# vita-epfl/CrowdNav

Measured on NVIDIA H100. Metric: env-steps/sec at 5 humans × batched envs; 500-case success/collision parity, higher is better.
Workload: dtype f64 state + f32 ORCA solver

## Files before the change

crowdnav_b200/csrc/reset_kernel.cu:

```cuda
#include <limits.h>
#include "scene.cuh"

namespace cs {

__device__ __forceinline__ bool next_seed(const crowdsim_reset_args &a, int e, const int *assigned, uint32_t &seed, int &case_id)
{
    if (a.case_counter) {
        const int c = assigned ? assigned[e] : atomicAdd(a.case_counter, 1);
        if (c >= a.case_total) return false;
        seed = queue_seed(a, c); case_id = c;
        return true;
    }
    seed = a.seed[e];
    if (a.seed_stride) a.seed[e] = seed + a.seed_stride;
    case_id = -1;
    return true;
}

struct ResetKArgs {
    crowdsim_reset_args a;
    crowdsim_state st;
    crowdsim_episodes ep;
    crowdsim_autoreset ar;
    int has_ep, B, N;
    int *assigned;
};

__device__ __forceinline__ void reset_env(const ResetKArgs &A, int e, MT &rng)
{
    const crowdsim_reset_args &a = A.a;
    const int N = A.N;
    uint32_t seed; int case_id;
    if (!next_seed(a, e, A.assigned, seed, case_id)) {
        if (A.st.active) A.st.active[e] = 0;
        if (A.has_ep) A.ep.ep_case[e] = -1;
        return;
    }
    rng.seed(seed);
    double *hp = A.st.h_pos + (size_t)e * N * 2, *hv = A.st.h_vel + (size_t)e * N * 2;
    double *hg = A.st.h_goal + (size_t)e * N * 2, *ha = A.st.h_attr + (size_t)e * N * 2;
    st2(A.st.r_pos, e, make_double2(0.0, -a.circle_radius)); st2(A.st.r_goal, e, make_double2(0.0, a.circle_radius));
    st2(A.st.r_vel, e, make_double2(0, 0)); st2(A.st.r_attr, e, make_double2(a.robot_radius, a.robot_v_pref));
    if (A.st.r_theta) A.st.r_theta[e] = CS_PI / 2;
    A.st.g_time[e] = 0.0;
    generate_scene(rng, a, N, hp, hg, ha);
    for (int i = 0; i < N; ++i) { hv[2 * i] = 0.0; hv[2 * i + 1] = 0.0; }
    if (A.st.active) A.st.active[e] = 1;
    if (A.has_ep) {
        A.ep.ep_steps[e] = 0; A.ep.ep_return[e] = 0.0; A.ep.ep_too_close[e] = 0; A.ep.ep_min_dist_sum[e] = 0.0;
        if (a.case_counter) A.ep.ep_case[e] = case_id;
    }
}

__device__ __forceinline__ void prefetch_env(const ResetKArgs &A, int e, MT &rng)
{
    const crowdsim_autoreset &ar = A.ar;
    const int N = A.N;
    uint32_t seed; int case_id;
    if (!next_seed(A.a, e, A.assigned, seed, case_id)) {
        ar.n_case[e] = -1;
        st_release_u8(ar.n_state + e, CROWDSIM_SLOT_EXHAUSTED);
        return;
    }
    rng.seed(seed);
    generate_scene(rng, A.a, N, ar.n_h_pos + (size_t)e * N * 2, ar.n_h_goal + (size_t)e * N * 2, ar.n_h_attr + (size_t)e * N * 2);
    ar.n_case[e] = case_id;
    st_release_u8(ar.n_state + e, CROWDSIM_SLOT_READY);
}

template <bool PREFETCH>
__global__ void __launch_bounds__(32, 32) scene_kernel(const __grid_constant__ ResetKArgs A)
{
    CS_RES_BEGIN
    const int lane = threadIdx.x, base = blockIdx.x * 32, e = base + lane;
    const bool need = e < A.B && (PREFETCH ? ld_acquire_u8(A.ar.n_state + e) == (A.assigned ? CROWDSIM_SLOT_CLAIMED : CROWDSIM_SLOT_EMPTY)
                                           : !(A.a.mask && !A.a.mask[e]));
    const unsigned bal = __ballot_sync(0xffffffffu, need);
    MT rng; rng.mt = A.a.scene_mt + base + lane; rng.stride = A.B;
    for (int k = lane; k < __popc(bal); k += 32) {
        const int slot = base + (int)__fns(bal, 0, k + 1);
        if (PREFETCH) prefetch_env(A, slot, rng); else reset_env(A, slot, rng);
    }
#ifdef CS_RESIDENCY_PROBE
    __syncwarp();
#endif
    CS_RES_END(CS_RES_SCENE);
}

constexpr int kAssignThreads = 64;
constexpr int kAssignRun = 32;
template <bool PREFETCH>
__global__ void __launch_bounds__(kAssignThreads, 16) assign_cases_kernel(const __grid_constant__ ResetKArgs A)
{
    CS_RES_BEGIN
    __shared__ int s_warp[kAssignThreads / 32];
    const int tid = threadIdx.x, lane = tid & 31, w = tid >> 5;
    int base = *A.a.case_counter;
    for (int start = 0; start < A.B; start += kAssignThreads * kAssignRun) {
        const int e0 = start + tid * kAssignRun;
        uint8_t flag[kAssignRun];
        #pragma unroll
        for (int j = 0; j < kAssignRun; ++j) {
            const int e = e0 + j;
            flag[j] = 0;
            if (e < A.B) {
                if (PREFETCH) flag[j] = ld_relaxed_u8(A.ar.n_state + e) == CROWDSIM_SLOT_EMPTY;
                else flag[j] = !(A.a.mask && !A.a.mask[e]);
            }
        }
        if (PREFETCH) fence_acquire_gpu();
        unsigned need = 0;
        #pragma unroll
        for (int j = 0; j < kAssignRun; ++j) need |= (unsigned)flag[j] << j;
        const int cnt = __popc(need);
        int incl = cnt;
        #pragma unroll
        for (int d = 1; d < 32; d <<= 1) { const int t = __shfl_up_sync(0xffffffffu, incl, d); if (lane >= d) incl += t; }
        if (lane == 31) s_warp[w] = incl;
        __syncthreads();
        int next = base + incl - cnt;
        #pragma unroll
        for (int v = 0; v < kAssignThreads / 32; ++v) if (v < w) next += s_warp[v];
        int total = 0;
        #pragma unroll
        for (int v = 0; v < kAssignThreads / 32; ++v) total += s_warp[v];
        while (need) {
            const int j = __ffs(need) - 1;
            need &= need - 1u;
            A.assigned[e0 + j] = next++;
            if (PREFETCH) A.ar.n_state[e0 + j] = CROWDSIM_SLOT_CLAIMED;
        }
        base += total;
        __syncthreads();
    }
    if (tid == 0) *A.a.case_counter = base;
    CS_RES_END(CS_RES_ASSIGN);
}

template <bool PREFETCH>
static int launch_scene_kernel(ResetKArgs A, int B, cudaStream_t stream)
{
    cudaError_t err = set_carveout<scene_kernel<PREFETCH>>();
    if (err == cudaSuccess) err = set_carveout<assign_cases_kernel<PREFETCH>>();
    if (err != cudaSuccess) return (int)err;
    A.assigned = nullptr;
    if (A.a.case_counter && (PREFETCH || A.has_ep)) {
        A.assigned = PREFETCH ? A.ar.n_case : A.ep.ep_case;
        assign_cases_kernel<PREFETCH><<<1, kAssignThreads, 0, stream>>>(A);
        ++g_launches;
    }
    scene_kernel<PREFETCH><<<(B + 31) / 32, 32, 0, stream>>>(A);
    ++g_launches;
    return (int)cudaGetLastError();
}

}

#ifdef CS_RESIDENCY_PROBE
extern "C" int crowdsim_residency_probe_refill(cs::ResRec *out, unsigned cap, unsigned *n) { return cs::res_read(out, cap, n); }
#endif

static int check_reset_args(const crowdsim_reset_args *args, int B, int N)
{
    if (!args || B < 0 || N < 0) return CROWDSIM_EINVAL;
    if (!args->case_counter && !args->seed) return CROWDSIM_EINVAL;
    if (N > CROWDSIM_MAX_HUMANS) return CROWDSIM_EUNSUPPORTED;
    if (args->rule != CROWDSIM_RULE_CIRCLE && args->rule != CROWDSIM_RULE_SQUARE && args->rule != CROWDSIM_RULE_MIXED) return CROWDSIM_EUNSUPPORTED;
    if (args->rule == CROWDSIM_RULE_MIXED && N < 5) return CROWDSIM_EUNSUPPORTED;
    if (!args->scene_mt) return CROWDSIM_EINVAL;
    if (B > INT_MAX / 624) return CROWDSIM_EUNSUPPORTED;
    return CROWDSIM_OK;
}

extern "C" int crowdsim_reset(const crowdsim_reset_args *args, int B, int N, crowdsim_state *st, crowdsim_episodes *ep,
                              void *stream)
{
    if (!st) return CROWDSIM_EINVAL;
    if (int rc = check_reset_args(args, B, N)) return rc;
    if (N > 0 && (!st->h_pos || !st->h_vel || !st->h_goal || !st->h_attr)) return CROWDSIM_EINVAL;
    if (!st->r_pos || !st->r_vel || !st->r_goal || !st->r_attr || !st->g_time) return CROWDSIM_EINVAL;
    if (ep && (!ep->ep_steps || !ep->ep_return || !ep->ep_too_close || !ep->ep_min_dist_sum || !ep->ep_case)) return CROWDSIM_EINVAL;
    if (B == 0) return CROWDSIM_OK;
    cs::ResetKArgs A; A.a = *args; A.st = *st; A.has_ep = ep != nullptr; A.B = B; A.N = N;
    if (ep) A.ep = *ep; else memset(&A.ep, 0, sizeof(A.ep));
    memset(&A.ar, 0, sizeof(A.ar));
    return cs::launch_scene_kernel<false>(A, B, (cudaStream_t)stream);
}

extern "C" int crowdsim_prefetch_scenes(const crowdsim_reset_args *args, int B, int N, const crowdsim_autoreset *ar, void *stream)
{
    if (!ar) return CROWDSIM_EINVAL;
    if (int rc = check_reset_args(args, B, N)) return rc;
    if (!ar->n_state || !ar->n_case || !ar->want || (N > 0 && (!ar->n_h_pos || !ar->n_h_goal || !ar->n_h_attr))) return CROWDSIM_EINVAL;
    if (B == 0) return CROWDSIM_OK;
    cs::ResetKArgs A; A.a = *args; A.ar = *ar; A.has_ep = 0; A.B = B; A.N = N;
    memset(&A.st, 0, sizeof(A.st)); memset(&A.ep, 0, sizeof(A.ep));
    return cs::launch_scene_kernel<true>(A, B, (cudaStream_t)stream);
}
```

crowdnav_b200/csrc/scene.cuh:

```cuda
#pragma once
#include "crowdsim_common.cuh"

namespace cs {

struct MT {
    uint32_t *mt;
    int stride;
    int pos;
    bool first;
    uint32_t a, a1, m;
    __host__ __device__ __forceinline__ uint32_t &w(int i) { return mt[i * stride]; }
    static __host__ __device__ __forceinline__ uint32_t init_step(uint32_t s, int k) { return 1812433253u * (s ^ (s >> 30)) + (uint32_t)k; }
    __host__ __device__ void seed(uint32_t s) {
        a = s; a1 = init_step(s, 1);
        m = a1;
        for (int k = 2; k <= 397; ++k) m = init_step(m, k);
        pos = 0; first = true;
    }
    __host__ __device__ __forceinline__ void resume(int p) { pos = p; first = false; }
    __host__ __device__ void store_seeded() {
        if (!first) return;
        for (int i = pos; i < 624; ++i) { w(i) = a; a = init_step(a, i + 1); }
        first = false;
    }
    __host__ __device__ __forceinline__ uint32_t next() {
        const int i = pos;
        const int i1 = (i == 623) ? 0 : i + 1;
        const int im = (i < 227) ? i + 397 : i - 227;
        uint32_t wi, wi1, wm;
        if (first) { wi = a; wi1 = (i == 623) ? w(0) : a1; wm = (i < 227) ? m : w(im); }
        else { wi = w(i); wi1 = w(i1); wm = w(im); }
        const uint32_t y0 = (wi & 0x80000000u) | (wi1 & 0x7fffffffu);
        uint32_t y = wm ^ (y0 >> 1) ^ ((y0 & 1u) ? 0x9908b0dfu : 0u);
        w(i) = y;
        if (first) {
            a = a1; a1 = init_step(a1, i + 2); m = init_step(m, i + 398);
            first = i != 623;
        }
        pos = i1;
        y ^= (y >> 11); y ^= (y << 7) & 0x9d2c5680u; y ^= (y << 15) & 0xefc60000u; y ^= (y >> 18);
        return y;
    }
    __host__ __device__ __forceinline__ double next_double() {
        const uint32_t a_ = next() >> 5, b_ = next() >> 6;
        return (a_ * 67108864.0 + b_) / 9007199254740992.0;
    }
    __host__ __device__ __forceinline__ int next_index(uint32_t A) {
        const uint32_t rng = A - 1u;
        if (rng == 0u) return 0;
        uint32_t mask = rng;
        mask |= mask >> 1; mask |= mask >> 2; mask |= mask >> 4; mask |= mask >> 8; mask |= mask >> 16;
        uint32_t v;
        do { v = next() & mask; } while (v > rng);
        return (int)v;
    }
};

template <class RNG>
__host__ __device__ __forceinline__ void generate_scene(RNG &rng, const crowdsim_reset_args &a, int N, double *hp, double *hg, double *ha)
{
    const double rpx = 0.0, rpy = -a.circle_radius, rgx = 0.0, rgy = a.circle_radius;
    auto put = [&](int i, double px, double py, double gx, double gy, double radius, double v_pref) {
        hp[2 * i] = px; hp[2 * i + 1] = py; hg[2 * i] = gx; hg[2 * i + 1] = gy; ha[2 * i] = radius; ha[2 * i + 1] = v_pref;
    };
    auto attributes = [&](double &radius, double &v_pref) {
        radius = a.human_radius; v_pref = a.human_v_pref;
        if (a.randomize_attributes) {
            v_pref = 0.5 + (1.5 - 0.5) * rng.next_double();
            radius = 0.3 + (0.5 - 0.3) * rng.next_double();
        }
    };
    auto circle_human = [&](int i) {
        double radius, v_pref, px, py; attributes(radius, v_pref);
        for (;;) {
            const double angle = rng.next_double() * CS_PI * 2;
            const double px_noise = (rng.next_double() - 0.5) * v_pref;
            const double py_noise = (rng.next_double() - 0.5) * v_pref;
            px = a.circle_radius * cos(angle) + px_noise;
            py = a.circle_radius * sin(angle) + py_noise;
            bool collide = false;
            for (int k = -1; k < i && !collide; ++k) {
                const double ar = (k < 0) ? a.robot_radius : ha[2 * k];
                const double apx = (k < 0) ? rpx : hp[2 * k], apy = (k < 0) ? rpy : hp[2 * k + 1];
                const double agx = (k < 0) ? rgx : hg[2 * k], agy = (k < 0) ? rgy : hg[2 * k + 1];
                const double min_dist = radius + ar + a.discomfort_dist;
                if (norm2(px - apx, py - apy) < min_dist || norm2(px - agx, py - agy) < min_dist) collide = true;
            }
            if (!collide) break;
        }
        put(i, px, py, -px, -py, radius, v_pref);
    };
    auto square_human = [&](int i) {
        double radius, v_pref, px, py, gx, gy; attributes(radius, v_pref);
        const double sign = (rng.next_double() > 0.5) ? -1.0 : 1.0;
        for (;;) {
            px = rng.next_double() * a.square_width * 0.5 * sign;
            py = (rng.next_double() - 0.5) * a.square_width;
            bool collide = false;
            for (int k = -1; k < i && !collide; ++k) {
                const double ar = (k < 0) ? a.robot_radius : ha[2 * k];
                const double apx = (k < 0) ? rpx : hp[2 * k], apy = (k < 0) ? rpy : hp[2 * k + 1];
                if (norm2(px - apx, py - apy) < radius + ar + a.discomfort_dist) collide = true;
            }
            if (!collide) break;
        }
        for (;;) {
            gx = rng.next_double() * a.square_width * 0.5 * -sign;
            gy = (rng.next_double() - 0.5) * a.square_width;
            bool collide = false;
            for (int k = -1; k < i && !collide; ++k) {
                const double ar = (k < 0) ? a.robot_radius : ha[2 * k];
                const double agx = (k < 0) ? rgx : hg[2 * k], agy = (k < 0) ? rgy : hg[2 * k + 1];
                if (norm2(gx - agx, gy - agy) < radius + ar + a.discomfort_dist) collide = true;
            }
            if (!collide) break;
        }
        put(i, px, py, gx, gy, radius, v_pref);
    };
    if (a.rule == CROWDSIM_RULE_CIRCLE) { for (int i = 0; i < N; ++i) circle_human(i); return; }
    if (a.rule == CROWDSIM_RULE_SQUARE) { for (int i = 0; i < N; ++i) square_human(i); return; }
    const bool is_static = rng.next_double() < 0.2;
    double prob = rng.next_double();
    const double p_static[6] = {0.05, 0.2, 0.2, 0.3, 0.1, 0.15}, p_dynamic[6] = {0.0, 0.3, 0.3, 0.2, 0.1, 0.1};
    int count = N;
    for (int key = is_static ? 0 : 1; key <= 5; ++key) {
        const double value = is_static ? p_static[key] : p_dynamic[key];
        if (prob - value <= 0) { count = key; break; }
        prob -= value;
    }
    if (count > N) count = N;
    int placed = 0;
    if (is_static) {
        const double width = 4, height = 8;
        if (count == 0 && N > 0) { put(0, 0.0, -10.0, 0.0, -10.0, a.human_radius, a.human_v_pref); placed = 1; }
        for (int i = 0; i < count; ++i) {
            const double sign = (rng.next_double() > 0.5) ? -1.0 : 1.0;
            double px, py;
            for (;;) {
                px = rng.next_double() * width * 0.5 * sign;
                py = (rng.next_double() - 0.5) * height;
                bool collide = false;
                for (int k = -1; k < i && !collide; ++k) {
                    const double ar = (k < 0) ? a.robot_radius : ha[2 * k];
                    const double apx = (k < 0) ? rpx : hp[2 * k], apy = (k < 0) ? rpy : hp[2 * k + 1];
                    if (norm2(px - apx, py - apy) < a.human_radius + ar + a.discomfort_dist) collide = true;
                }
                if (!collide) break;
            }
            put(i, px, py, px, py, a.human_radius, a.human_v_pref);
        }
        if (count > 0) placed = count;
    } else {
        for (int i = 0; i < count; ++i) { if (i < 2) circle_human(i); else square_human(i); }
        placed = count;
    }
    for (int i = placed; i < N; ++i) {
        const double x = CROWDSIM_PARKED_X + 100.0 * i;
        put(i, x, CROWDSIM_PARKED_X, x, CROWDSIM_PARKED_X, a.human_radius, a.human_v_pref);
    }
}

__device__ __forceinline__ uint32_t queue_seed(const crowdsim_reset_args &a, int c)
{
    return a.seed_base + (a.case_wrap > 0 ? (uint32_t)(((long long)a.case_first + c) % a.case_wrap) : (uint32_t)c);
}

}
```

Baseline: 1.321 billion.

## Generate scenes in shared-memory scratch with a flattened rejection loop and wider blocks

After: 1.367 billion, median of 6. 3.5% higher.

```diff
diff --git a/crowdnav_b200/csrc/reset_kernel.cu b/crowdnav_b200/csrc/reset_kernel.cu
--- a/crowdnav_b200/csrc/reset_kernel.cu
+++ b/crowdnav_b200/csrc/reset_kernel.cu
@@ -26,7 +26,12 @@
     int *assigned;
 };
 
-__device__ __forceinline__ void reset_env(const ResetKArgs &A, int e, MT &rng)
+__device__ __forceinline__ void store_scene(const double *scratch, int N, double *hp, double *hg, double *ha)
+{
+    for (int j = 0; j < 2 * N; ++j) { hp[j] = scratch[j]; hg[j] = scratch[2 * N + j]; ha[j] = scratch[4 * N + j]; }
+}
+
+__device__ __forceinline__ void reset_env(const ResetKArgs &A, int e, MT &rng, double *scratch)
 {
     const crowdsim_reset_args &a = A.a;
     const int N = A.N;
@@ -43,7 +48,8 @@
     st2(A.st.r_vel, e, make_double2(0, 0)); st2(A.st.r_attr, e, make_double2(a.robot_radius, a.robot_v_pref));
     if (A.st.r_theta) A.st.r_theta[e] = CS_PI / 2;
     A.st.g_time[e] = 0.0;
-    generate_scene(rng, a, N, hp, hg, ha);
+    generate_scene(rng, a, N, scratch, scratch + 2 * N, scratch + 4 * N);
+    store_scene(scratch, N, hp, hg, ha);
     for (int i = 0; i < N; ++i) { hv[2 * i] = 0.0; hv[2 * i + 1] = 0.0; }
     if (A.st.active) A.st.active[e] = 1;
     if (A.has_ep) {
@@ -52,7 +58,7 @@
     }
 }
 
-__device__ __forceinline__ void prefetch_env(const ResetKArgs &A, int e, MT &rng)
+__device__ __forceinline__ void prefetch_env(const ResetKArgs &A, int e, MT &rng, double *scratch)
 {
     const crowdsim_autoreset &ar = A.ar;
     const int N = A.N;
@@ -63,23 +69,36 @@
         return;
     }
     rng.seed(seed);
-    generate_scene(rng, A.a, N, ar.n_h_pos + (size_t)e * N * 2, ar.n_h_goal + (size_t)e * N * 2, ar.n_h_attr + (size_t)e * N * 2);
+    generate_scene(rng, A.a, N, scratch, scratch + 2 * N, scratch + 4 * N);
+    store_scene(scratch, N, ar.n_h_pos + (size_t)e * N * 2, ar.n_h_goal + (size_t)e * N * 2, ar.n_h_attr + (size_t)e * N * 2);
     ar.n_case[e] = case_id;
     st_release_u8(ar.n_state + e, CROWDSIM_SLOT_READY);
 }
 
+constexpr int kSceneSlots = 48;
+static_assert(kSceneSlots >= 32 && kSceneSlots <= 64, "a scene block ballots its slots in two words");
+
+__host__ __device__ __forceinline__ int scene_scratch_stride(int N) { return 6 * N + 1; }
+
 template <bool PREFETCH>
 __global__ void __launch_bounds__(32, 32) scene_kernel(const __grid_constant__ ResetKArgs A)
 {
     CS_RES_BEGIN
-    const int lane = threadIdx.x, base = blockIdx.x * 32, e = base + lane;
-    const bool need = e < A.B && (PREFETCH ? ld_acquire_u8(A.ar.n_state + e) == (A.assigned ? CROWDSIM_SLOT_CLAIMED : CROWDSIM_SLOT_EMPTY)
-                                           : !(A.a.mask && !A.a.mask[e]));
-    const unsigned bal = __ballot_sync(0xffffffffu, need);
+    extern __shared__ double s_scene[];
+    const int lane = threadIdx.x, base = blockIdx.x * kSceneSlots;
+    auto need = [&](int j) {
+        const int e = base + j;
+        if (j >= kSceneSlots || e >= A.B) return false;
+        return PREFETCH ? ld_acquire_u8(A.ar.n_state + e) == (A.assigned ? CROWDSIM_SLOT_CLAIMED : CROWDSIM_SLOT_EMPTY)
+                        : !(A.a.mask && !A.a.mask[e]);
+    };
+    const unsigned lo = __ballot_sync(0xffffffffu, need(lane)), hi = __ballot_sync(0xffffffffu, need(32 + lane));
+    const int n_lo = __popc(lo), n = n_lo + __popc(hi);
     MT rng; rng.mt = A.a.scene_mt + base + lane; rng.stride = A.B;
-    for (int k = lane; k < __popc(bal); k += 32) {
-        const int slot = base + (int)__fns(bal, 0, k + 1);
-        if (PREFETCH) prefetch_env(A, slot, rng); else reset_env(A, slot, rng);
+    double *scratch = s_scene + (size_t)lane * scene_scratch_stride(A.N);
+    for (int k = lane; k < n; k += 32) {
+        const int slot = base + (k < n_lo ? (int)__fns(lo, 0, k + 1) : 32 + (int)__fns(hi, 0, k - n_lo + 1));
+        if (PREFETCH) prefetch_env(A, slot, rng, scratch); else reset_env(A, slot, rng, scratch);
     }
 #ifdef CS_RESIDENCY_PROBE
     __syncwarp();
@@ -149,7 +168,12 @@
         assign_cases_kernel<PREFETCH><<<1, kAssignThreads, 0, stream>>>(A);
         ++g_launches;
     }
-    scene_kernel<PREFETCH><<<(B + 31) / 32, 32, 0, stream>>>(A);
+    const size_t smem = (size_t)32 * scene_scratch_stride(A.N) * sizeof(double);
+    if (smem > 48 * 1024) {
+        err = cudaFuncSetAttribute(scene_kernel<PREFETCH>, cudaFuncAttributeMaxDynamicSharedMemorySize, (int)smem);
+        if (err != cudaSuccess) return (int)err;
+    }
+    scene_kernel<PREFETCH><<<(B + kSceneSlots - 1) / kSceneSlots, 32, smem, stream>>>(A);
     ++g_launches;
     return (int)cudaGetLastError();
 }
diff --git a/crowdnav_b200/csrc/scene.cuh b/crowdnav_b200/csrc/scene.cuh
--- a/crowdnav_b200/csrc/scene.cuh
+++ b/crowdnav_b200/csrc/scene.cuh
@@ -63,96 +63,74 @@
     auto put = [&](int i, double px, double py, double gx, double gy, double radius, double v_pref) {
         hp[2 * i] = px; hp[2 * i + 1] = py; hg[2 * i] = gx; hg[2 * i + 1] = gy; ha[2 * i] = radius; ha[2 * i + 1] = v_pref;
     };
-    auto attributes = [&](double &radius, double &v_pref) {
-        radius = a.human_radius; v_pref = a.human_v_pref;
-        if (a.randomize_attributes) {
-            v_pref = 0.5 + (1.5 - 0.5) * rng.next_double();
-            radius = 0.3 + (0.5 - 0.3) * rng.next_double();
+    bool is_static = false;
+    int count = N, placed = N;
+    if (a.rule == CROWDSIM_RULE_MIXED) {
+        is_static = rng.next_double() < 0.2;
+        double prob = rng.next_double();
+        const double p_static[6] = {0.05, 0.2, 0.2, 0.3, 0.1, 0.15}, p_dynamic[6] = {0.0, 0.3, 0.3, 0.2, 0.1, 0.1};
+        for (int key = is_static ? 0 : 1; key <= 5; ++key) {
+            const double value = is_static ? p_static[key] : p_dynamic[key];
+            if (prob - value <= 0) { count = key; break; }
+            prob -= value;
         }
+        if (count > N) count = N;
+        placed = count;
+        if (is_static && count == 0 && N > 0) { put(0, 0.0, -10.0, 0.0, -10.0, a.human_radius, a.human_v_pref); placed = 1; }
+    }
+    enum { kCircle, kSquare, kStatic };
+    auto kind_of = [&](int i) {
+        if (a.rule == CROWDSIM_RULE_CIRCLE) return (int)kCircle;
+        if (a.rule == CROWDSIM_RULE_SQUARE) return (int)kSquare;
+        return is_static ? (int)kStatic : (i < 2 ? (int)kCircle : (int)kSquare);
     };
-    auto circle_human = [&](int i) {
-        double radius, v_pref, px, py; attributes(radius, v_pref);
-        for (;;) {
+    double radius = 0, v_pref = 0, sign = 0, px = 0, py = 0;
+    auto collides = [&](int i, double x, double y, bool pos, bool goal) {
+        for (int k = -1; k < i; ++k) {
+            const double ar = (k < 0) ? a.robot_radius : ha[2 * k];
+            const double min_dist = radius + ar + a.discomfort_dist;
+            if (pos) {
+                const double apx = (k < 0) ? rpx : hp[2 * k], apy = (k < 0) ? rpy : hp[2 * k + 1];
+                if (norm2(x - apx, y - apy) < min_dist) return true;
+            }
+            if (goal) {
+                const double agx = (k < 0) ? rgx : hg[2 * k], agy = (k < 0) ? rgy : hg[2 * k + 1];
+                if (norm2(x - agx, y - agy) < min_dist) return true;
+            }
+        }
+        return false;
+    };
+    int stage = 0;
+    for (int i = 0; i < count;) {
+        const int kind = kind_of(i);
+        if (stage == 0) {
+            radius = a.human_radius; v_pref = a.human_v_pref;
+            if (kind != kStatic && a.randomize_attributes) {
+                v_pref = 0.5 + (1.5 - 0.5) * rng.next_double();
+                radius = 0.3 + (0.5 - 0.3) * rng.next_double();
+            }
+            if (kind != kCircle) sign = (rng.next_double() > 0.5) ? -1.0 : 1.0;
+            stage = 1;
+        }
+        if (kind == kCircle) {
             const double angle = rng.next_double() * CS_PI * 2;
             const double px_noise = (rng.next_double() - 0.5) * v_pref;
             const double py_noise = (rng.next_double() - 0.5) * v_pref;
-            px = a.circle_radius * cos(angle) + px_noise;
-            py = a.circle_radius * sin(angle) + py_noise;
-            bool collide = false;
-            for (int k = -1; k < i && !collide; ++k) {
-                const double ar = (k < 0) ? a.robot_radius : ha[2 * k];
-                const double apx = (k < 0) ? rpx : hp[2 * k], apy = (k < 0) ? rpy : hp[2 * k + 1];
-                const double agx = (k < 0) ? rgx : hg[2 * k], agy = (k < 0) ? rgy : hg[2 * k + 1];
-                const double min_dist = radius + ar + a.discomfort_dist;
-                if (norm2(px - apx, py - apy) < min_dist || norm2(px - agx, py - agy) < min_dist) collide = true;
+            double sin_a, cos_a;
+            sincos(angle, &sin_a, &cos_a);
+            px = a.circle_radius * cos_a + px_noise;
+            py = a.circle_radius * sin_a + py_noise;
+            if (!collides(i, px, py, true, true)) { put(i, px, py, -px, -py, radius, v_pref); ++i; stage = 0; }
+        } else {
+            const bool goal = stage == 2;
+            const double width = kind == kStatic ? 4.0 : a.square_width, height = kind == kStatic ? 8.0 : a.square_width;
+            const double x = rng.next_double() * width * 0.5 * (goal ? -sign : sign);
+            const double y = (rng.next_double() - 0.5) * height;
+            if (!collides(i, x, y, !goal, goal)) {
+                if (kind == kSquare && !goal) { px = x; py = y; stage = 2; }
+                else { put(i, goal ? px : x, goal ? py : y, x, y, radius, v_pref); ++i; stage = 0; }
             }
-            if (!collide) break;
         }
-        put(i, px, py, -px, -py, radius, v_pref);
-    };
-    auto square_human = [&](int i) {
-        double radius, v_pref, px, py, gx, gy; attributes(radius, v_pref);
-        const double sign = (rng.next_double() > 0.5) ? -1.0 : 1.0;
-        for (;;) {
-            px = rng.next_double() * a.square_width * 0.5 * sign;
-            py = (rng.next_double() - 0.5) * a.square_width;
-            bool collide = false;
-            for (int k = -1; k < i && !collide; ++k) {
-                const double ar = (k < 0) ? a.robot_radius : ha[2 * k];
-                const double apx = (k < 0) ? rpx : hp[2 * k], apy = (k < 0) ? rpy : hp[2 * k + 1];
-                if (norm2(px - apx, py - apy) < radius + ar + a.discomfort_dist) collide = true;
-            }
-            if (!collide) break;
-        }
-        for (;;) {
-            gx = rng.next_double() * a.square_width * 0.5 * -sign;
-            gy = (rng.next_double() - 0.5) * a.square_width;
-            bool collide = false;
-            for (int k = -1; k < i && !collide; ++k) {
-                const double ar = (k < 0) ? a.robot_radius : ha[2 * k];
-                const double agx = (k < 0) ? rgx : hg[2 * k], agy = (k < 0) ? rgy : hg[2 * k + 1];
-                if (norm2(gx - agx, gy - agy) < radius + ar + a.discomfort_dist) collide = true;
-            }
-            if (!collide) break;
-        }
-        put(i, px, py, gx, gy, radius, v_pref);
-    };
-    if (a.rule == CROWDSIM_RULE_CIRCLE) { for (int i = 0; i < N; ++i) circle_human(i); return; }
-    if (a.rule == CROWDSIM_RULE_SQUARE) { for (int i = 0; i < N; ++i) square_human(i); return; }
-    const bool is_static = rng.next_double() < 0.2;
-    double prob = rng.next_double();
-    const double p_static[6] = {0.05, 0.2, 0.2, 0.3, 0.1, 0.15}, p_dynamic[6] = {0.0, 0.3, 0.3, 0.2, 0.1, 0.1};
-    int count = N;
-    for (int key = is_static ? 0 : 1; key <= 5; ++key) {
-        const double value = is_static ? p_static[key] : p_dynamic[key];
-        if (prob - value <= 0) { count = key; break; }
-        prob -= value;
-    }
-    if (count > N) count = N;
-    int placed = 0;
-    if (is_static) {
-        const double width = 4, height = 8;
-        if (count == 0 && N > 0) { put(0, 0.0, -10.0, 0.0, -10.0, a.human_radius, a.human_v_pref); placed = 1; }
-        for (int i = 0; i < count; ++i) {
-            const double sign = (rng.next_double() > 0.5) ? -1.0 : 1.0;
-            double px, py;
-            for (;;) {
-                px = rng.next_double() * width * 0.5 * sign;
-                py = (rng.next_double() - 0.5) * height;
-                bool collide = false;
-                for (int k = -1; k < i && !collide; ++k) {
-                    const double ar = (k < 0) ? a.robot_radius : ha[2 * k];
-                    const double apx = (k < 0) ? rpx : hp[2 * k], apy = (k < 0) ? rpy : hp[2 * k + 1];
-                    if (norm2(px - apx, py - apy) < a.human_radius + ar + a.discomfort_dist) collide = true;
-                }
-                if (!collide) break;
-            }
-            put(i, px, py, px, py, a.human_radius, a.human_v_pref);
-        }
-        if (count > 0) placed = count;
-    } else {
-        for (int i = 0; i < count; ++i) { if (i < 2) circle_human(i); else square_human(i); }
-        placed = count;
     }
     for (int i = placed; i < N; ++i) {
         const double x = CROWDSIM_PARKED_X + 100.0 * i;
```
